# rdesc/autorally

Measured on AMD Instinct MI355X. Metric: trajectory rollouts/s per MPPI solve, higher is better.
Workload: dtype f32

## Files before the change

### autorally_amd/csrc/group_roles.hpp

```cpp
#pragma once

#include "mppi_device.hpp"
#include "noise_device.hpp"

namespace mppi {

constexpr int kGRing = 16;
constexpr int kGCtlChunk = 4;

template <class SH>
struct GroupRoles {
  static constexpr int kPose = SH::NW, kCost = SH::NW + 1, kCtl = SH::NW + 2, kRng = SH::NW + 3;
  static constexpr int kWaves = SH::NW + 4;
  static_assert(kWaves <= (int)(sizeof(SH::fin) / sizeof(int)), "fin[]");
  static_assert(SH::kR == 16 || SH::kR == 8, "rollouts per group");
};
template <class SH>
__device__ __forceinline__ int group_j(int slot) { return slot & (SH::kR - 1); }
template <class SH>
__device__ __forceinline__ bool group_real(int slot) { return slot < SH::kR; }

template <class SH>
__device__ __forceinline__ int group_seq_min(SH &sh)
{
  int m = lds_peek(lds_addr(&sh.xseq[0][0]));
#pragma unroll
  for (int w = 1; w < SH::NW; w++) m = min(m, lds_peek(lds_addr(&sh.xseq[w][0])));
  return m;
}

struct MrgHalf {
  uint32_t s0, s1, s2;
};
__device__ __forceinline__ uint32_t fold_m(uint64_t x, uint32_t C, uint32_t m)
{
  x = (x >> 32) * C + (x & 0xffffffffULL);
  x = (x >> 32) * C + (x & 0xffffffffULL);
  x = (x >> 32) * C + (x & 0xffffffffULL);
  if (x >= m) x -= m;
  return (uint32_t)x;
}
template <class SH>
__device__ __forceinline__ MrgHalf group_rng_load(const RolloutArgs &a)
{
  const int lane = threadIdx.x & 63;
  const int j = group_j<SH>((lane >> 1) & 15), c = lane & 1;
  const int k = (int)blockIdx.x * SH::kR + j;
  const int K = a.K;
  MrgHalf g{0, 0, 0};
  if (a.inline_noise != 0 && lane < 2 * kRolloutsPerWave) {
    g.s0 = a.rng_in[(3 * c) * K + k]; g.s1 = a.rng_in[(3 * c + 1) * K + k]; g.s2 = a.rng_in[(3 * c + 2) * K + k];
  }
  return g;
}
template <class SH, bool PRE = false>
__device__ __forceinline__ void group_rng_wave(const RolloutArgs &a, SH &sh, const MrgHalf pre = MrgHalf{0, 0, 0})
{
  using R = GroupRoles<SH>;
  const int lane = threadIdx.x & 63;
  const int j = group_j<SH>((lane >> 1) & 15), c = lane & 1;
  const int k = (int)blockIdx.x * SH::kR + j;
  const int K = a.K, T = a.T;
  const bool active = lane < 2 * kRolloutsPerWave;
  const bool real = lane < 2 * SH::kR;
  int budget = spin_budget_init(a.spin_budget, T, a.fault_wave == R::kRng + 1);
  if (a.inline_noise != 0) {
    const uint32_t m = c ? (uint32_t)kM2 : (uint32_t)kM1, C = c ? kC2 : kC1;
    const uint32_t A = c ? (uint32_t)kA21 : (uint32_t)kA12, Bn = c ? (uint32_t)kA23N : (uint32_t)kA13N;
    MrgHalf g{0, 0, 0};
    if constexpr (PRE) {
      g = pre;
    } else if (active) {
      g.s0 = a.rng_in[(3 * c) * K + k]; g.s1 = a.rng_in[(3 * c + 1) * K + k]; g.s2 = a.rng_in[(3 * c + 2) * K + k];
    }
    const uint32_t a_ctl = lds_addr(&sh.ctl_pub[0]);
    const uint32_t a_mypub = lds_addr(&sh.rng_pub[lane]);
    int seen = 0;
    for (int t = 0; t < T; t++) {
      float2 e = make_float2(0.5f, 0.5f);
#ifdef MPPI_DIAG_NORNG
      e = make_float2(0.25f + 0.001f * (float)t, 0.5f);
#else
#pragma unroll
      for (int d = 0; d < 2; d++) {
        const uint32_t p = fold_m((uint64_t)A * (c ? g.s2 : g.s1) + (uint64_t)Bn * (m - g.s0), C, m);
        g.s0 = g.s1; g.s1 = g.s2; g.s2 = p;
        const uint32_t p2 = (uint32_t)__builtin_amdgcn_mov_dpp((int)p, 0xB1, 0xF, 0xF, false);
        uint32_t z = (p >= p2) ? p - p2 : p + (uint32_t)kM1 - p2;
        if (z == 0) z = (uint32_t)kM1;
        const float u = (float)z * 0x1p-32f;
        if (d == 0) e.x = u; else e.y = u;
      }
#endif
      const int need = t - kGRing + 1;
      while (seen < need && --budget > 0) {
        seen = lds_peek(a_ctl);
        if (seen < need) __builtin_amdgcn_s_sleep(2);
      }
      if (active && c == 0) *reinterpret_cast<float2 *>(&sh.eps[t & (kGRing - 1)][j][0]) = e;
      lds_publish(a_mypub, t + 1);
    }
    if (real) {
      a.rng_out[(3 * c) * K + k] = g.s0; a.rng_out[(3 * c + 1) * K + k] = g.s1; a.rng_out[(3 * c + 2) * K + k] = g.s2;
    }
  }
  spin_finish(budget, lds_addr(&sh.fail[0]), lds_addr(&sh.fin[R::kRng]));
}

template <class SH>
__device__ __forceinline__ void group_control_wave(const RolloutArgs &a, SH &sh, const uint32_t a_gate_open = 0)
{
  using R = GroupRoles<SH>;
  constexpr int NSW = SH::NSW;
  static_assert(kGCtlChunk == 4 && kGRing >= 2 * kGCtlChunk, "four steps per iteration, lanes 16 q + j");
  const int lane = threadIdx.x & 63;
  const int j = group_j<SH>(lane & 15), q = lane >> 4;
  const bool real = group_real<SH>(lane & 15);
  const int k = (int)blockIdx.x * SH::kR + j;
  const int K = a.K, T = a.T;
  const bool inl = a.inline_noise != 0;
  float2 *const noise = reinterpret_cast<float2 *>(a.noise);
  const float2 *const Useq = reinterpret_cast<const float2 *>(a.U);
  const bool noise_free_k = (k == 0);
  const bool pure_noise_k = (k >= a.k99);
  const uint32_t a_cd = lds_addr(&sh.cost_done[0]);
  const uint32_t a_mypub = lds_addr(&sh.ctl_pub[lane]);
  const uint32_t a_rng = lds_addr(&sh.rng_pub[0]);
  int budget = spin_budget_init(a.spin_budget, T, a.fault_wave == R::kCtl + 1);
  const bool gated = a_gate_open != 0;
  if (gated)
    while (lds_peek(a_gate_open) == 0 && --budget > 0) __builtin_amdgcn_s_sleep(1);
  int seen_x = 0, seen_c = 0, seen_r = 0;
  for (int t0 = 0, n = 1; t0 < T; t0 += n, n = kGCtlChunk) {
    const int t = t0 + q;
    const bool live = (t < T) & (q < n);
    const int tl = live ? t : T - 1;
    float2 Ut;
    if (gated) {
      const unsigned long long ub = __hip_atomic_load(reinterpret_cast<const unsigned long long *>(Useq + tl), __ATOMIC_RELAXED, __HIP_MEMORY_SCOPE_SYSTEM);
      Ut = make_float2(__uint_as_float((unsigned)ub), __uint_as_float((unsigned)(ub >> 32)));
    } else {
      Ut = Useq[tl];
    }
    float2 e = (live && !inl) ? noise[(size_t)tl * K + k] : make_float2(0.0f, 0.0f);
    const int tm = min(t0 + n, T) - 1;
    const int need_x = (tm >= kGRing) ? (tm - kGRing) * NSW + 1 : 0;
    const int need_c = tm - kGRing + 1;
    while ((seen_x < need_x || seen_c < need_c) && --budget > 0) {
      seen_x = group_seq_min(sh);
      seen_c = lds_peek(a_cd);
      if (seen_x < need_x || seen_c < need_c) __builtin_amdgcn_s_sleep(2);
    }
    if (inl) {
      while (seen_r < tm + 1 && --budget > 0) {
        seen_r = lds_peek(a_rng);
        if (seen_r < tm + 1) __builtin_amdgcn_s_sleep(1);
      }
#ifdef MPPI_DIAG_NOBM
      e = *reinterpret_cast<const float2 *>(&sh.eps[tl & (kGRing - 1)][j][0]);
#else
      e = box_muller(*reinterpret_cast<const float2 *>(&sh.eps[tl & (kGRing - 1)][j][0]));
#endif
    }
    if (live) {
      const bool nf = noise_free_k | (t < a.opt_delay);
      const float n0 = e.x * a.nu[0], n1 = e.y * a.nu[1];
      const float du0 = nf ? 0.0f : n0, du1 = nf ? 0.0f : n1;
      float u0 = nf ? Ut.x : (pure_noise_k ? n0 : Ut.x + n0);
      float u1 = nf ? Ut.y : (pure_noise_k ? n1 : Ut.y + n1);
      if (real) noise[(size_t)t * K + k] = make_float2(u0, u1);
      u0 = clampf(u0, a.u_lo[0], a.u_hi[0]);
      u1 = clampf(u1, a.u_lo[1], a.u_hi[1]);
      const int slot = t & (kGRing - 1);
      sh.ctl_b1[slot][j] = u0;
      sh.ctl_b1[slot][kRolloutsPerWave + j] = u1;
      *reinterpret_cast<float4 *>(&sh.ctl_rec[slot][j][0]) = make_float4(u0, u1, du0, du1);
    }
    lds_publish(a_mypub, tm + 1);
  }
  spin_finish(budget, lds_addr(&sh.fail[0]), lds_addr(&sh.fin[R::kCtl]));
}

template <class SH, bool AFFINE>
__device__ __forceinline__ void group_pose_wave(const RolloutArgs &a, SH &sh)
{
  using R = GroupRoles<SH>;
  constexpr int NSW = SH::NSW;
  static_assert(SH::kR == 16, "one step per iteration: 16-rollout groups only");
  const int lane = threadIdx.x & 63;
  const int j = lane & 15;
  const int T = a.T;
  const uint32_t a_seq0 = lds_addr(&sh.xseq[0][0]);
  const uint32_t a_cd = lds_addr(&sh.cost_done[0]);
  const uint32_t a_mypub = lds_addr(&sh.pose_pub[lane]);
  float x = a.state[0], y = a.state[1], yaw = a.state[2];
  int budget = spin_budget_init(a.spin_budget, T, a.fault_wave == R::kPose + 1), seen = 0, cdone = 0;
  float tf_p = 0.0f, tb_p = 0.0f;
  for (int t = 0; t <= T; t++) {
    float tf = 0.0f, tb = 0.0f;
    if (t < T) {
      const int need = t * NSW + 1;
      while (seen < need && --budget > 0) {
        seen = SH::kRecByAll ? group_seq_min(sh) : lds_peek(a_seq0);
        if (seen < need) __builtin_amdgcn_s_sleep(1);
      }
      const float4 r0 = *reinterpret_cast<const float4 *>(&sh.rec[t & (kGRing - 1)][j][0]);
      float spsi, cpsi;
#ifdef MPPI_DIAG_NOPOSE
      spsi = 0.0f; cpsi = 1.0f; tf = x; tb = y;
#else
      sincos_fast(yaw, spsi, cpsi);
      const float st[3] = {x, y, yaw};
      track_fetch<AFFINE>(a.cost, st, cpsi, spsi, tf, tb);
#endif
      const float sd0 = fmaf(cpsi, r0.y, -(spsi * r0.z));
      const float sd1 = fmaf(spsi, r0.y, cpsi * r0.z);
      const float sd2 = a.negate_yaw_der ? -r0.w : r0.w;
      x = fmaf(sd0, a.dt, x);
      y = fmaf(sd1, a.dt, y);
      yaw = fmaf(sd2, a.dt, yaw);
    }
    if (t > 0) {
      while (cdone < t - kGRing && --budget > 0) cdone = lds_peek(a_cd);
      if (lane < kRolloutsPerWave) *reinterpret_cast<float2 *>(&sh.tex[(t - 1) & (kGRing - 1)][lane][0]) = make_float2(tf_p, tb_p);
      lds_publish(a_mypub, t);
    }
    tf_p = tf; tb_p = tb;
  }
  spin_finish(budget, lds_addr(&sh.fail[0]), lds_addr(&sh.fin[R::kPose]));
}

template <int Q>
__device__ __forceinline__ float quad_bc(float v)
{
  return __int_as_float(__builtin_amdgcn_mov_dpp(__float_as_int(v), Q * 0x55, 0xF, 0xF, false));
}
__device__ __forceinline__ void quad_chain(float v, float d, float dt, int q, float &vq, float &v_out)
{
  const float v1 = fmaf(quad_bc<0>(d), dt, v);
  const float v2 = fmaf(quad_bc<1>(d), dt, v1);
  const float v3 = fmaf(quad_bc<2>(d), dt, v2);
  v_out = fmaf(quad_bc<3>(d), dt, v3);
  const float lo = (q == 0) ? v : v1, hi = (q == 2) ? v2 : v3;
  vq = (q < 2) ? lo : hi;
}
template <class SH, bool AFFINE>
__device__ __forceinline__ void group_pose_wave4(const RolloutArgs &a, SH &sh, const float x0, const float y0, const float yaw0,
                                                 const int budget_cut = 0);
template <class SH, bool AFFINE>
__device__ __forceinline__ void group_pose_wave4(const RolloutArgs &a, SH &sh)
{
  group_pose_wave4<SH, AFFINE>(a, sh, a.state[0], a.state[1], a.state[2]);
}
template <class SH, bool AFFINE>
__device__ __forceinline__ void group_pose_wave4(const RolloutArgs &a, SH &sh, const float x0, const float y0, const float yaw0,
                                                 const int budget_cut)
{
  using R = GroupRoles<SH>;
  constexpr int NSW = SH::NSW;
  static_assert(kRolloutsPerWave == 16 && kGRing >= 8, "lane = 4 j + q");
  const int lane = threadIdx.x & 63;
  const int j = group_j<SH>(lane >> 2), q = lane & 3;
  const int T = a.T;
  const uint32_t a_seq0 = lds_addr(&sh.xseq[0][0]);
  const uint32_t a_cd = lds_addr(&sh.cost_done[0]);
  const uint32_t a_mypub = lds_addr(&sh.pose_pub[lane]);
  float x = x0, y = y0, yaw = yaw0;
  int budget = spin_budget_init(a.spin_budget, T, a.fault_wave == R::kPose + 1 || budget_cut != 0), seen = 0, cdone = 0;
  for (int t0 = 0; t0 < T; t0 += 4) {
    const int t = t0 + q;
    const int tend = min(t0 + 4, T);
    const int need = (tend - 1) * NSW + 1;
    while (seen < need && --budget > 0) {
      seen = SH::kRecByAll ? group_seq_min(sh) : lds_peek(a_seq0);
      if (seen < need) __builtin_amdgcn_s_sleep(1);
    }
    const float4 r0 = *reinterpret_cast<const float4 *>(&sh.rec[t & (kGRing - 1)][j][0]);
    float yaw_q, yaw_n, x_q, x_n, y_q, y_n;
    quad_chain(yaw, a.negate_yaw_der ? -r0.w : r0.w, a.dt, q, yaw_q, yaw_n);
    float spsi, cpsi, tf = 0.0f, tb = 0.0f;
#ifdef MPPI_DIAG_NOPOSE
    spsi = 0.0f; cpsi = 1.0f;
#else
    sincos_fast(yaw_q, spsi, cpsi);
#endif
    quad_chain(x, fmaf(cpsi, r0.y, -(spsi * r0.z)), a.dt, q, x_q, x_n);
    quad_chain(y, fmaf(spsi, r0.y, cpsi * r0.z), a.dt, q, y_q, y_n);
#ifdef MPPI_DIAG_NOPOSE
    tf = x_q; tb = y_q;
#else
    const float st[3] = {x_q, y_q, yaw_q};
    track_fetch<AFFINE>(a.cost, st, cpsi, spsi, tf, tb);
#endif
    x = x_n; y = y_n; yaw = yaw_n;
    while (cdone < tend - kGRing && --budget > 0) cdone = lds_peek(a_cd);
    if (t < T) *reinterpret_cast<float2 *>(&sh.tex[t & (kGRing - 1)][j][0]) = make_float2(tf, tb);
    lds_publish(a_mypub, tend);
  }
  spin_finish(budget, lds_addr(&sh.fail[0]), lds_addr(&sh.fin[R::kPose]));
}

template <class SH>
__device__ __forceinline__ float group_settle(SH &sh, int budget, float J)
{
  using R = GroupRoles<SH>;
  const int lane = threadIdx.x & 63;
  const uint32_t a_fin = lds_addr(&sh.fin[(lane < R::kWaves) ? lane : 0]);
  for (;;) {
    const int v = (lane == R::kCost) ? 1 : lds_peek_lanes(a_fin);
    const bool all = __builtin_amdgcn_ballot_w64(v != 0) == ~0ull;
    if (all || --budget <= 0) break;
    __builtin_amdgcn_s_sleep(1);
  }
  if (budget <= 0 || lds_peek(lds_addr(&sh.fail[0])) != 0) J = __builtin_nanf("");
  return J;
}

template <class SH, bool CTRL>
__device__ __forceinline__ void group_cost_wave(const RolloutArgs &a, SH &sh)
{
  using R = GroupRoles<SH>;
  const int lane = threadIdx.x & 63;
  static_assert(SH::kR == 16, "one step per iteration: 16-rollout groups only");
  const int j = lane & 15;
  const int k = (int)blockIdx.x * kRolloutsPerWave + j;
  const int T = a.T;
  const uint32_t a_mydone = lds_addr(&sh.cost_done[lane]);
  const uint32_t a_pose = lds_addr(&sh.pose_pub[0]);
  int crash = 0, budget = spin_budget_init(a.spin_budget, T, a.fault_wave == R::kCost + 1), seen = 0;
  float J = 0.0f;
  for (int t = 0; t < T; t++) {
    const double rt = a.inv_t[t];
    while (seen < t + 1 && --budget > 0) {
      seen = lds_peek(a_pose);
      if (seen < t + 1) __builtin_amdgcn_s_sleep(1);
    }
    const float4 r0 = *reinterpret_cast<const float4 *>(&sh.rec[t & (kGRing - 1)][j][0]);
    const float4 r1 = *reinterpret_cast<const float4 *>(&sh.ctl_rec[t & (kGRing - 1)][j][0]);
    const float2 tx = *reinterpret_cast<const float2 *>(&sh.tex[t & (kGRing - 1)][j][0]);
    lds_publish(a_mydone, t + 1);
    const int rc = (int)((t > 0) & (fabsf(r0.x) >= kRollCrash));
#ifdef MPPI_DIAG_NOCOST
    crash |= rc;
    int crash_new = crash;
    const float Jn = J + r0.y + r1.x + tx.x + (float)rt;
#else
    CostTerms ct;
    cost_terms_a<CTRL>(a.cost, a.nu, r0.y, r0.z, r1.x, r1.y, r1.z, r1.w, ct);
    crash |= rc;
    int crash_new = crash;
    const float c = cost_terms_b(a.cost, ct, tx.x, tx.y, crash_new);
    const float Jn = running_mean(J, c, t, rt);
#endif
    J = (t > 0) ? Jn : J;
    crash = (t > 0) ? crash_new : crash;
  }
  J = group_settle(sh, budget, J);
  a.costs[k] = J + 0.0f;
}

template <int Q>
__device__ __forceinline__ int quad_bc_i(int v)
{
  return __builtin_amdgcn_mov_dpp(v, Q * 0x55, 0xF, 0xF, false);
}
template <class SH, bool CTRL>
__device__ __forceinline__ void group_cost_wave4(const RolloutArgs &a, SH &sh)
{
  using R = GroupRoles<SH>;
  const int lane = threadIdx.x & 63;
  const int j = group_j<SH>(lane >> 2), q = lane & 3;
  const int k = (int)blockIdx.x * SH::kR + j;
  const int T = a.T;
  const uint32_t a_mydone = lds_addr(&sh.cost_done[lane]);
  const uint32_t a_pose = lds_addr(&sh.pose_pub[0]);
  int crash = 0, budget = spin_budget_init(a.spin_budget, T, a.fault_wave == R::kCost + 1), seen = 0;
  float J = 0.0f;
  for (int t0 = 0; t0 < T; t0 += 4) {
    const int t = t0 + q;
    const int tend = min(t0 + 4, T);
    while (seen < tend && --budget > 0) {
      seen = lds_peek(a_pose);
      if (seen < tend) __builtin_amdgcn_s_sleep(1);
    }
    const float4 r0 = *reinterpret_cast<const float4 *>(&sh.rec[t & (kGRing - 1)][j][0]);
    const float4 r1 = *reinterpret_cast<const float4 *>(&sh.ctl_rec[t & (kGRing - 1)][j][0]);
    const float2 tx = *reinterpret_cast<const float2 *>(&sh.tex[t & (kGRing - 1)][j][0]);
    lds_publish(a_mydone, tend);
    const bool counted = (t > 0) & (t < T);
    int e = (int)(fabsf(r0.x) >= kRollCrash) | (int)(tx.x >= a.cost.boundary_threshold) | (int)(tx.y >= a.cost.boundary_threshold);
    e = counted ? e : 0;
    const int c0 = crash | quad_bc_i<0>(e), c1 = c0 | quad_bc_i<1>(e), c2 = c1 | quad_bc_i<2>(e), c3 = c2 | quad_bc_i<3>(e);
    const int lo = (q == 0) ? c0 : c1, hi = (q == 2) ? c2 : c3;
    int crash_q = (q < 2) ? lo : hi;
    crash = c3;
#ifdef MPPI_DIAG_NOCOST
    const float c = r0.y + r1.x + tx.x + (float)crash_q;
#else
    CostTerms ct;
    cost_terms_a<CTRL>(a.cost, a.nu, r0.y, r0.z, r1.x, r1.y, r1.z, r1.w, ct);
    const float c = cost_terms_b(a.cost, ct, tx.x, tx.y, crash_q);
#endif
#pragma unroll
    for (int l = 0; l < 4; l++) {
      const int tl = t0 + l;
      const float cl = (l == 0) ? quad_bc<0>(c) : (l == 1) ? quad_bc<1>(c) : (l == 2) ? quad_bc<2>(c) : quad_bc<3>(c);
      if (tl > 0 && tl < T) {
#ifdef MPPI_DIAG_NOCOST
        J = J + cl + (float)a.inv_t[tl];
#else
        J = running_mean(J, cl, tl, a.inv_t[tl]);
#endif
      }
    }
  }
  J = group_settle(sh, budget, J);
  if (q == 0 && group_real<SH>(lane >> 2)) a.costs[k] = J + 0.0f;
}

}
```

### autorally_amd/csrc/mppi_device.hpp

```cpp
#pragma once

#include <hip/hip_runtime.h>
#include <stdint.h>

namespace mppi {

constexpr int kStateDim = 7;
constexpr int kControlDim = 2;
constexpr int kNetIn = 6;
constexpr int kNetOut = 4;
constexpr int kRolloutsPerWave = 16;

struct CostArgs {
  float desired_speed, speed_coeff, track_coeff, max_slip_ang, slip_penalty, track_slop;
  float crash_coeff, steering_coeff, throttle_coeff, boundary_threshold;
  float crash_cost_discounted;
  int l1_cost;
  float r_c1[3], r_c2[3], trs[3];
  int affine;
  int need_control_cost;
  int map_w, map_h;
  const float *map;
};

struct RolloutArgs {
  float state[kStateDim];
  const float *U;
  float *noise;
  float *costs;
  const float *wpack;
  const double *inv_t;
  const uint32_t *rng_in;
  uint32_t *rng_out;
  int inline_noise;
  int K, T, opt_delay, k99;
  float nu[2], u_lo[2], u_hi[2], dt;
  int negate_yaw_der;
  int spin_budget, fault_wave;
  const unsigned *gate;
  unsigned gate_seq;
  unsigned gate_ticks;
  unsigned long long *min_cost;
  unsigned min_cost_tag;
  CostArgs cost;
};
constexpr int kGateReplicas = 8;
constexpr int kGateUOffset = 16 * kGateReplicas;
inline int gate_hist_offset(int T) { return kGateUOffset + 2 * T; }
inline size_t gate_block_floats(int T) { return (size_t)gate_hist_offset(T) + 4; }
constexpr unsigned kGateCancel = 0x80000000u;

constexpr int kMinCostLines = 8, kMinCostStride = 16;
__device__ __forceinline__ unsigned cost_order_bits(float x)
{
  const unsigned b = __float_as_uint(x);
  return b ^ ((b >> 31) ? 0xFFFFFFFFu : 0x80000000u);
}
__device__ __forceinline__ float cost_from_order_bits(unsigned o)
{
  return __uint_as_float(o ^ ((o >> 31) ? 0x80000000u : 0xFFFFFFFFu));
}
template <int CTRL>
__device__ __forceinline__ float wave_dpp(float v)
{
  return __int_as_float(__builtin_amdgcn_update_dpp(0, __float_as_int(v), CTRL, 0xF, 0xF, true));
}
template <bool MIN>
__device__ __forceinline__ float wave_reduce(float v)
{
#define MPPI_RED(A, B) (MIN ? fminf((A), (B)) : (A) + (B))
  v = MPPI_RED(v, wave_dpp<0xB1>(v));
  v = MPPI_RED(v, wave_dpp<0x4E>(v));
  v = MPPI_RED(v, wave_dpp<0x141>(v));
  v = MPPI_RED(v, wave_dpp<0x140>(v));
  const auto x = __builtin_amdgcn_permlane16_swap(__float_as_uint(v), __float_as_uint(v), false, false);
  v = MPPI_RED(__uint_as_float(x[0]), __uint_as_float(x[1]));
  const auto y = __builtin_amdgcn_permlane32_swap(__float_as_uint(v), __float_as_uint(v), false, false);
  v = MPPI_RED(__uint_as_float(y[0]), __uint_as_float(y[1]));
#undef MPPI_RED
  return v;
}
__device__ __forceinline__ void publish_min_cost(const RolloutArgs &a, const float mine)
{
  if (a.min_cost == nullptr) return;
  const float m = wave_reduce<true>((mine == mine) ? mine : INFINITY);
  if ((threadIdx.x & 63) == 0 && m < INFINITY) {
    const unsigned long long key = ((unsigned long long)(~a.min_cost_tag) << 32) | cost_order_bits(m);
    (void)__hip_atomic_fetch_min(a.min_cost + (blockIdx.x % kMinCostLines) * kMinCostStride, key, __ATOMIC_RELAXED, __HIP_MEMORY_SCOPE_AGENT);
  }
}
__device__ __forceinline__ bool load_min_cost(const unsigned long long *min_cost, const unsigned tag, float &beta)
{
  if (min_cost == nullptr) return false;
  unsigned long long k[kMinCostLines];
#pragma unroll
  for (int i = 0; i < kMinCostLines; i++) k[i] = __hip_atomic_load(min_cost + i * kMinCostStride, __ATOMIC_RELAXED, __HIP_MEMORY_SCOPE_AGENT);
  unsigned long long best = k[0];
#pragma unroll
  for (int i = 1; i < kMinCostLines; i++) best = (k[i] < best) ? k[i] : best;
  beta = cost_from_order_bits((unsigned)best);
  return (unsigned)(best >> 32) == ~tag;
}

constexpr int kMaxBatch = 4;
template <int NB>
struct QuadBatchArgsT {
  int n;
  RolloutArgs inst[NB];
};
using QuadBatchArgs = QuadBatchArgsT<kMaxBatch>;
template <int NB>
inline QuadBatchArgsT<NB> batch_args_prefix(const QuadBatchArgs &b)
{
  QuadBatchArgsT<NB> s;
  s.n = b.n;
  for (int i = 0; i < NB; i++) s.inst[i] = b.inst[i];
  return s;
}
static_assert(kMaxBatch == 4, "MPPI_BATCH_DISPATCH");
#define MPPI_BATCH_DISPATCH(NB, B, BODY)     \
  do {                                      \
    if constexpr ((NB) == 2) {              \
      if (blockIdx.y == 0) BODY((B).inst[0]); \
      else BODY((B).inst[1]);               \
    } else {                                \
      switch ((int)blockIdx.y) {            \
        case 0: BODY((B).inst[0]); break;   \
        case 1: BODY((B).inst[1]); break;   \
        case 2: BODY((B).inst[2]); break;   \
        default: BODY((B).inst[3]); break;  \
      }                                     \
    }                                       \
  } while (0)

template <class T>
__device__ __forceinline__ T *load_global_ptr(T *const &field)
{
  using G = __attribute__((address_space(1))) T *;
  return (T *)*static_cast<const G *>(static_cast<const void *>(&field));
}

__device__ constexpr float kRollCrash = 1.57000005245208740234375f;
__device__ constexpr float kMinSpeed = 0.001000000047497451305389404296875f;
__device__ constexpr float kCostCapGt = 1000000061440.0f;
__device__ constexpr float kCostCap = 999999995904.0f;

__device__ __forceinline__ float clampf(float v, float lo, float hi)
{
  float r = (v > hi) ? hi : v;
  r = (v < lo) ? lo : r;
  return r;
}

__device__ __forceinline__ float tanh_fast(float x)
{
  const float e = __builtin_amdgcn_exp2f(x * 2.88539008177792681472f);
  const float r = __builtin_amdgcn_rcpf(e + 1.0f);
  return fmaf(-2.0f, r, 1.0f);
}

constexpr float kTanhScale = 2.88539008177792681472f;
__device__ __forceinline__ float tanh_bias(float z, float bs)
{
  const float e = __builtin_amdgcn_exp2f(fmaf(z, kTanhScale, bs));
  const float r = __builtin_amdgcn_rcpf(e + 1.0f);
  return fmaf(-2.0f, r, 1.0f);
}

typedef float f32x2 __attribute__((ext_vector_type(2)));
typedef float f32x4 __attribute__((ext_vector_type(4)));
__device__ __forceinline__ f32x2 tanh_bias2(f32x2 z, f32x2 bs)
{
  const f32x2 y = __builtin_elementwise_fma(z, f32x2{kTanhScale, kTanhScale}, bs);
  f32x2 e;
  e.x = __builtin_amdgcn_exp2f(y.x);
  e.y = __builtin_amdgcn_exp2f(y.y);
  const f32x2 d = e + f32x2{1.0f, 1.0f};
  f32x2 r;
  r.x = __builtin_amdgcn_rcpf(d.x);
  r.y = __builtin_amdgcn_rcpf(d.y);
  return __builtin_elementwise_fma(f32x2{-2.0f, -2.0f}, r, f32x2{1.0f, 1.0f});
}

__device__ __forceinline__ void sincos_fast(float x, float &sn, float &cs)
{
  const double xd = (double)x;
  const double q = rint(xd * 0.63661977236758134308);
  double rd = fma(-q, 1.5707963267948966, xd);
  rd = fma(-q, 6.123233995736766e-17, rd);
  const float r = (float)rd;
  const float r2 = r * r;
  const float ps = fmaf(fmaf(-1.9515295891e-4f, r2, 8.3321608736e-3f), r2, -1.6666654611e-1f);
  const float s0 = fmaf(r * r2, ps, r);
  const float pc = fmaf(fmaf(2.443315711809948e-5f, r2, -1.388731625493765e-3f), r2, 4.166664568298827e-2f);
  const float c0 = fmaf(r2 * r2, pc, fmaf(r2, -0.5f, 1.0f));
  const int qi = (int)q;
  const float a = (qi & 1) ? c0 : s0;
  const float b = (qi & 1) ? s0 : c0;
  sn = (qi & 2) ? -a : a;
  cs = ((qi + 1) & 2) ? -b : b;
}

template <bool AFFINE>
__device__ __forceinline__ unsigned texel_index(const CostArgs &c, float x, float y)
{
  float u = fmaf(c.r_c1[0], x, c.r_c2[0] * y) + c.trs[0];
  float v = fmaf(c.r_c1[1], x, c.r_c2[1] * y) + c.trs[1];
  if (!AFFINE) {
    const float w = fmaf(c.r_c1[2], x, c.r_c2[2] * y) + c.trs[2];
    u = u / w;
    v = v / w;
  }
  float fi = floorf(u * (float)c.map_w);
  float fj = floorf(v * (float)c.map_h);
  fi = fminf(fmaxf(fi, 0.0f), (float)(c.map_w - 1));
  fj = fminf(fmaxf(fj, 0.0f), (float)(c.map_h - 1));
  return (unsigned)((int)fj * c.map_w + (int)fi);
}

template <bool AFFINE>
__device__ __forceinline__ void track_fetch(const CostArgs &c, const float *s, float cpsi, float spsi,
                                            float &tf, float &tb)
{
  const float xf = fmaf(0.5f, cpsi, s[0]), yf = fmaf(0.5f, spsi, s[1]);
  const float xb = fmaf(-0.5f, cpsi, s[0]), yb = fmaf(-0.5f, spsi, s[1]);
  tf = c.map[texel_index<AFFINE>(c, xf, yf)];
  tb = c.map[texel_index<AFFINE>(c, xb, yb)];
}

struct CostTerms {
  float control_cost, speed_cost, stabilizing_cost;
};

template <bool CTRL_COST>
__device__ __forceinline__ void cost_terms_a(const CostArgs &c, const float nu[2], float s4, float s5,
                                             float u0, float u1, float du0, float du1, CostTerms &o)
{
  float control_cost = 0.0f;
  if (CTRL_COST) {
    control_cost += c.steering_coeff * du0 * (u0 - du0) / (nu[0] * nu[0]);
    control_cost += c.throttle_coeff * du1 * (u1 - du1) / (nu[1] * nu[1]);
  }
  o.control_cost = control_cost;
  const float err = s4 - c.desired_speed;
  o.speed_cost = c.speed_coeff * (c.l1_cost ? fabsf(err) : err * err);
  const float slip = -atanf(s5 / fabsf(s4));
  float stab = c.slip_penalty * (slip * slip);
  stab = (fabsf(slip) > c.max_slip_ang) ? stab + c.crash_coeff : stab;
  o.stabilizing_cost = (fabsf(s4) >= kMinSpeed) ? stab : 0.0f;
}

__device__ __forceinline__ float cost_terms_b(const CostArgs &c, const CostTerms &a, float tf, float tb,
                                              int &crash)
{
  float track_cost = (fabsf(tf) + fabsf(tb)) * 0.5f;
  track_cost = (fabsf(track_cost) < c.track_slop) ? 0.0f : c.track_coeff * track_cost;
  crash |= (int)(tf >= c.boundary_threshold) | (int)(tb >= c.boundary_threshold);
  const float crash_cost = (crash > 0) ? c.crash_cost_discounted : 0.0f;
  float cost = a.control_cost + a.speed_cost + crash_cost + track_cost + a.stabilizing_cost;
  cost = (cost >= kCostCapGt || cost != cost) ? kCostCap : cost;
  return cost;
}

template <bool CTRL_COST>
__device__ __forceinline__ float cost_finish(const CostArgs &c, const float nu[2], float s4, float s5,
                                             float tf, float tb, float u0, float u1, float du0,
                                             float du1, int &crash)
{
  CostTerms t;
  cost_terms_a<CTRL_COST>(c, nu, s4, s5, u0, u1, du0, du1, t);
  return cost_terms_b(c, t, tf, tb, crash);
}

__device__ __forceinline__ float running_mean(float J, float c, int t, double rt)
{
  const double d = (double)(c - J);
  const double td = (double)t;
  const double q0 = d * rt;
  const double e = fma(-q0, td, d);
  const double q = fma(e, rt, q0);
  return (float)((double)J + q);
}

constexpr int kSpinBudget = 1 << 22;

__device__ __forceinline__ uint32_t lds_addr(const void *p)
{
  return (uint32_t)(uintptr_t)(const __attribute__((address_space(3))) void *)p;
}
__device__ __forceinline__ void lds_publish(uint32_t addr, int v)
{
  asm volatile("ds_write_b32 %0, %1" ::"v"(addr), "v"(v) : "memory");
}
__device__ __forceinline__ void lds_put4(uint32_t addr, f32x4 v)
{
  asm volatile("ds_write_b128 %0, %1" ::"v"(addr), "v"(v) : "memory");
}
__device__ __forceinline__ int lds_peek(uint32_t addr)
{
  int v;
  asm volatile("ds_read_b32 %0, %1\n\ts_waitcnt lgkmcnt(0)" : "=&v"(v) : "v"(addr) : "memory");
  return __builtin_amdgcn_readfirstlane(v);
}
__device__ __forceinline__ void lds_pin_reads() { asm volatile("" ::: "memory"); }
__device__ __forceinline__ float row_sel(int g, float s3, float s4, float s5, float s6)
{
  const float lo = (g == 0) ? s3 : s4;
  const float hi = (g == 2) ? s5 : s6;
  return (g < 2) ? lo : hi;
}

__device__ __forceinline__ int lds_peek_lanes(uint32_t addr)
{
  int v;
  asm volatile("ds_read_b32 %0, %1\n\ts_waitcnt lgkmcnt(0)" : "=&v"(v) : "v"(addr) : "memory");
  return v;
}

__device__ __forceinline__ int spin_budget_init(int spin_budget, int T, bool inject_fault)
{
  if (inject_fault) return 0;
  return (spin_budget > 0 ? spin_budget : kSpinBudget) + 64 * T;
}
__device__ __forceinline__ void spin_finish(int budget, uint32_t a_fail, uint32_t a_fin)
{
  if (budget <= 0) lds_publish(a_fail, 1);
  lds_publish(a_fin, 1);
}

template <class SH>
__device__ __forceinline__ int group_gate_wait(const RolloutArgs &a, SH &sh)
{
  const int lane = threadIdx.x & 63;
  const unsigned *blk = a.gate + (size_t)((int)blockIdx.x % kGateReplicas) * 16;
  const unsigned long long t0 = __builtin_amdgcn_s_memrealtime();
  unsigned v = 0;
  for (;;) {
    v = __hip_atomic_load(blk + 7, __ATOMIC_RELAXED, __HIP_MEMORY_SCOPE_SYSTEM);
    if ((v & ~kGateCancel) == a.gate_seq) break;
    if (__builtin_amdgcn_s_memrealtime() - t0 > (unsigned long long)a.gate_ticks) { v = kGateCancel; break; }
    __builtin_amdgcn_s_sleep(2);
  }
  asm volatile("" ::: "memory");
  const float sv = __uint_as_float(__hip_atomic_load(blk + (lane & 7), __ATOMIC_RELAXED, __HIP_MEMORY_SCOPE_SYSTEM));
  if (lane < 7) sh.gstate[lane] = sv;
  lds_publish(lds_addr(&sh.gate_open[0]), 1);
  return (v & kGateCancel) ? 1 : 0;
}


}
```

### autorally_amd/csrc/rollout_row.hip

```cpp
#include "group_roles.hpp"
#include "mppi_kernels.hpp"

namespace mppi {

#ifdef MPPI_ROW_STAMPS
__device__ unsigned long long g_row_stamps[16];
#define RSTAMP(i)                                                                                         \
  do {                                                                                                    \
    if (blockIdx.x == 0 && (threadIdx.x & 63) == 0) {                                                     \
      unsigned long long t__;                                                                             \
      asm volatile("s_memtime %0\n\ts_waitcnt lgkmcnt(0)" : "=s"(t__)::"memory");                           \
      g_row_stamps[i] = t__;                                                                              \
    }                                                                                                     \
  } while (0)
#else
#define RSTAMP(i) do { } while (0)
#endif

template <int H>
struct RowShared {
  static constexpr int NW = 4;
  static constexpr int NSW = 1;
  static constexpr bool kRecByAll = true;
  static constexpr int kR = 16;
  int xseq[NW][64];
  float rec[kGRing][kRolloutsPerWave][4];
  int cost_done[64];
  float ctl_b1[kGRing][64];
  float ctl_rec[kGRing][kRolloutsPerWave][4];
  int ctl_pub[64];
  float tex[kGRing][kRolloutsPerWave][2];
  int pose_pub[64];
  float eps[kGRing][kRolloutsPerWave][2];
  int rng_pub[64];
  int fail[4];
  int fin[8];
  float gstate[8];
  int gate_open[8];
  float dump[NW][64 * 2 + (kGRing - 1) * kRolloutsPerWave * 4];
};

template <int H, bool TREE>
struct RowWeights {
  f32x2 w1[kNetIn], w2[H], w3[TREE ? 4 : H];
  f32x2 b1s, b2s, b3;
};

constexpr int kRowPackEntries = 40;
template <int H, bool TREE>
__device__ __forceinline__ void row_load(const float *rowpack, int p, RowWeights<H, TREE> &W)
{
  static_assert(H == 32, "entry layout of pack_row_weights");
  const float4 *pk = reinterpret_cast<const float4 *>(rowpack) + p;
#pragma unroll
  for (int i = 0; i < 3; i++) {
    const float4 v = pk[i * 16];
    W.w1[2 * i] = f32x2{v.x, v.y};
    W.w1[2 * i + 1] = f32x2{v.z, v.w};
  }
#pragma unroll
  for (int i = 0; i < H / 2; i++) {
    const float4 v = pk[(3 + i) * 16];
    W.w2[2 * i] = f32x2{v.x, v.y};
    W.w2[2 * i + 1] = f32x2{v.z, v.w};
    if constexpr (!TREE) {
      const float4 u = pk[(3 + H / 2 + i) * 16];
      W.w3[2 * i] = f32x2{u.x, u.y};
      W.w3[2 * i + 1] = f32x2{u.z, u.w};
    }
  }
  const float4 b = pk[35 * 16];
  W.b1s = f32x2{b.x, b.y};
  W.b2s = f32x2{b.z, b.w};
  if constexpr (TREE) {
    const float4 u = pk[37 * 16], v = pk[38 * 16], c = pk[39 * 16];
    W.w3[0] = f32x2{u.x, u.y};
    W.w3[1] = f32x2{u.z, u.w};
    W.w3[2] = f32x2{v.x, v.y};
    W.w3[3] = f32x2{v.z, v.w};
    W.b3 = f32x2{c.x, c.y};
  } else {
    const float4 c = pk[36 * 16];
    W.b3 = f32x2{c.x, c.y};
  }
}

template <int Q>
__device__ __forceinline__ float row_bc(float a)
{
  return __int_as_float(__builtin_amdgcn_mov_dpp(__float_as_int(a), 0x150 + Q, 0xF, 0xF, false));
}
template <int Q>
__device__ __forceinline__ f32x2 row_bc2(f32x2 a)
{
  return __builtin_bit_cast(f32x2, (long long)__builtin_amdgcn_mov_dpp(__builtin_bit_cast(long long, a), 0x150 + Q, 0xF, 0xF, false));
}
template <int Q>
__device__ __forceinline__ void row_dot_step(f32x2 &z, f32x2 &b, const f32x2 *w, f32x2 a)
{
  z = __builtin_elementwise_fma(w[2 * Q], f32x2{b.x, b.x}, z);
  __builtin_amdgcn_sched_barrier(0);
  const f32x2 bn = row_bc2<(Q + 1 < 16 ? Q + 1 : 15)>(a);
  __builtin_amdgcn_sched_barrier(0);
  z = __builtin_elementwise_fma(w[2 * Q + 1], f32x2{b.y, b.y}, z);
  __builtin_amdgcn_sched_barrier(0);
  b = bn;
}
__device__ __forceinline__ f32x2 row_dot_bc(const f32x2 *w, f32x2 a)
{
  f32x2 z = {0.0f, 0.0f};
  f32x2 b = row_bc2<0>(a);
  __builtin_amdgcn_sched_barrier(0);
#define RD4(Q) row_dot_step<Q>(z, b, w, a); row_dot_step<Q + 1>(z, b, w, a); row_dot_step<Q + 2>(z, b, w, a); row_dot_step<Q + 3>(z, b, w, a);
  RD4(0) RD4(4) RD4(8) RD4(12)
#undef RD4
  return z;
}

template <int CTRL>
__device__ __forceinline__ float dpp_add(float acc, float src)
{
  return acc + __int_as_float(__builtin_amdgcn_update_dpp(0, __float_as_int(src), CTRL, 0xF, 0xF, true));
}
__device__ __forceinline__ float row_out_tree(const f32x2 *w3, f32x2 a)
{
  const f32x2 ax = {a.x, a.x}, ay = {a.y, a.y};
  const f32x2 v01 = __builtin_elementwise_fma(w3[1], ay, w3[0] * ax);
  const f32x2 v23 = __builtin_elementwise_fma(w3[3], ay, w3[2] * ax);
  float v0 = dpp_add<0x128>(v01.x, v23.x);
  const float v1 = dpp_add<0x128>(v01.y, v23.y);
  v0 = dpp_add<0x141>(v0, v1);
  v0 = dpp_add<0xB1>(v0, v0);
  v0 = dpp_add<0x4E>(v0, v0);
  return v0;
}

template <int H, bool TREE, int Q>
__device__ __forceinline__ void row_step(const RolloutArgs &a, const RowWeights<H, TREE> &W, f32x2 &sp, f32x2 &un, const int t0,
                                         const uint32_t a_rec, const uint32_t a_myseq, const volatile int __attribute__((address_space(3))) *p_pub,
                                         const volatile f32x2 __attribute__((address_space(3))) *&pu,
                                         const volatile f32x2 __attribute__((address_space(3))) *p_u0, int &cp, int &budget)
{
  constexpr int kSlotF2 = kRolloutsPerWave * 2;
  constexpr uint32_t kRecStride = sizeof(float) * kRolloutsPerWave * 4;
  const int t = t0 + Q;
  const f32x2 u = un;
  const f32x2 slo = TREE ? f32x2{row_bc<0>(sp.x), row_bc<4>(sp.x)} : f32x2{row_bc<0>(sp.x), row_bc<0>(sp.y)};
  const f32x2 shi = TREE ? f32x2{row_bc<8>(sp.x), row_bc<12>(sp.x)} : f32x2{row_bc<1>(sp.x), row_bc<1>(sp.y)};
  if constexpr (TREE) asm volatile("ds_write_b32 %0, %1 offset:%2" ::"v"(a_rec), "v"(sp.x), "n"(Q * kRecStride) : "memory");
  else asm volatile("ds_write_b64 %0, %1 offset:%2" ::"v"(a_rec), "v"(sp), "n"(Q * kRecStride) : "memory");
  if constexpr (Q == 3) lds_publish(a_myseq, t + 1);
  f32x2 z = {0.0f, 0.0f};
  z = __builtin_elementwise_fma(W.w1[0], f32x2{slo.x, slo.x}, z);
  z = __builtin_elementwise_fma(W.w1[1], f32x2{slo.y, slo.y}, z);
  z = __builtin_elementwise_fma(W.w1[2], f32x2{shi.x, shi.x}, z);
  z = __builtin_elementwise_fma(W.w1[3], f32x2{shi.y, shi.y}, z);
  z = __builtin_elementwise_fma(W.w1[4], f32x2{u.x, u.x}, z);
  z = __builtin_elementwise_fma(W.w1[5], f32x2{u.y, u.y}, z);
  int cp_v = 0;
  if constexpr (Q == 0) cp_v = *p_pub;
  if constexpr (Q == 3) pu = p_u0 + ((t + 1) & (kGRing - 1)) * kSlotF2;
  constexpr int kUn = (Q == 3) ? 0 : (Q + 1) * kSlotF2;
  un = pu[kUn];
  const f32x2 a0 = tanh_bias2(z, W.b1s);
  const f32x2 a1 = tanh_bias2(row_dot_bc(W.w2, a0), W.b2s);
  const int want = t + 2;
  if constexpr (Q == 0) cp = __builtin_amdgcn_readfirstlane(cp_v);
  asm volatile("" : "+v"(un));
  if constexpr (TREE) {
    const float d = row_out_tree(W.w3, a1) + W.b3.x;
    sp.x = fmaf(d, a.dt, sp.x);
    asm volatile("" : "+v"(sp.x));
  } else {
    const f32x2 d = row_dot_bc(W.w3, a1) + W.b3;
    sp = __builtin_elementwise_fma(d, f32x2{a.dt, a.dt}, sp);
    asm volatile("" : "+v"(sp));
  }
  if (__builtin_expect(cp < want, 0)) {
    while (cp < want && --budget > 0) {
      cp = __builtin_amdgcn_readfirstlane(*p_pub);
      un = pu[kUn];
    }
    asm volatile("" : "+v"(un));
  }
}

template <int H, bool TREE, bool GATED = false>
__device__ __forceinline__ void row_dynamics(const RolloutArgs &a, RowShared<H> &sh, const int w)
{
  static_assert(H == 32, "row_dot_bc: 32 activations, two per lane of a 16-lane row");
  static_assert(kGRing % 4 == 0, "aligned chunks of four steps inside the ring");
  const int lane = threadIdx.x & 63;
  const int r = lane >> 4, p = lane & 15;
  const int jr = 4 * w + r;
  const bool odd = (p & 1) != 0;
  const int T = a.T;
  RowWeights<H, TREE> W;
  row_load<H, TREE>(a.wpack, p, W);
#pragma unroll
  for (int k = 0; k < H; k++) asm volatile("" : "+v"(W.w2[k]));
#pragma unroll
  for (int k = 0; k < (TREE ? 4 : H); k++) asm volatile("" : "+v"(W.w3[k]));

  const uint32_t a_myseq = lds_addr(&sh.xseq[w][lane]);
  typedef const volatile int __attribute__((address_space(3))) *lds_int_p;
  typedef const volatile f32x2 __attribute__((address_space(3))) *lds_f2_p;
  const lds_int_p p_pub = (lds_int_p)&sh.ctl_pub[0];
  uint32_t a_u0 = lds_addr(&sh.ctl_rec[0][jr][0]);
  asm volatile("" : "+v"(a_u0));
  const lds_f2_p p_u = (lds_f2_p)a_u0;
  const uint32_t a_rec0 = TREE ? (((p & 3) == 0) ? lds_addr(&sh.rec[0][jr][p >> 2]) : lds_addr(&sh.dump[w][2 * lane]))
                               : ((p < 2) ? lds_addr(&sh.rec[0][jr][2 * p]) : lds_addr(&sh.dump[w][2 * lane]));
  constexpr uint32_t kRecStride = sizeof(float) * kRolloutsPerWave * 4;

  int budget = spin_budget_init(a.spin_budget, T, a.fault_wave == w + 1);
  f32x2 sp;
  if constexpr (GATED) {
    const uint32_t a_go = lds_addr(&sh.gate_open[0]);
    while (lds_peek(a_go) == 0 && --budget > 0) __builtin_amdgcn_s_sleep(1);
    const volatile float *gs = sh.gstate;
    sp = TREE ? f32x2{gs[3 + (p >> 2)], 0.0f} : odd ? f32x2{gs[5], gs[6]} : f32x2{gs[3], gs[4]};
  } else {
    sp = TREE ? f32x2{a.state[3 + (p >> 2)], 0.0f} : odd ? f32x2{a.state[5], a.state[6]} : f32x2{a.state[3], a.state[4]};
  }
  if (w == 0) RSTAMP(2);
  int cp = 0;
  while ((cp = __builtin_amdgcn_readfirstlane(*p_pub)) < 1 && --budget > 0) __builtin_amdgcn_s_sleep(1);
  if (w == 0) RSTAMP(3);
  lds_f2_p pu = p_u;
  f32x2 un = pu[0];
  asm volatile("" : "+v"(un));

  const int NS = T - 1;
  for (int t0 = 0; t0 < NS; t0 += 4) {
    const uint32_t a_rec = a_rec0 + (uint32_t)(t0 & (kGRing - 1)) * kRecStride;
    row_step<H, TREE, 0>(a, W, sp, un, t0, a_rec, a_myseq, p_pub, pu, p_u, cp, budget);
    if (t0 + 1 >= NS) break;
    row_step<H, TREE, 1>(a, W, sp, un, t0, a_rec, a_myseq, p_pub, pu, p_u, cp, budget);
    if (t0 + 2 >= NS) break;
    row_step<H, TREE, 2>(a, W, sp, un, t0, a_rec, a_myseq, p_pub, pu, p_u, cp, budget);
    if (t0 + 3 >= NS) break;
    row_step<H, TREE, 3>(a, W, sp, un, t0, a_rec, a_myseq, p_pub, pu, p_u, cp, budget);
  }
  if (w == 0) RSTAMP(4);
  {
    const int t = T - 1;
    if constexpr (TREE) asm volatile("ds_write_b32 %0, %1" ::"v"(a_rec0 + (uint32_t)(t & (kGRing - 1)) * kRecStride), "v"(sp.x) : "memory");
    else asm volatile("ds_write_b64 %0, %1" ::"v"(a_rec0 + (uint32_t)(t & (kGRing - 1)) * kRecStride), "v"(sp) : "memory");
    lds_publish(a_myseq, t + 1);
  }
  spin_finish(budget, lds_addr(&sh.fail[0]), lds_addr(&sh.fin[w]));
}

template <int H, bool AFFINE, bool CTRL, bool TREE, bool GATED = false>
__device__ __forceinline__ void row_group(const RolloutArgs &a, RowShared<H> &sh)
{
  using SH = RowShared<H>;
  using R = GroupRoles<SH>;
  const int lane = threadIdx.x & 63;
  const int role = __builtin_amdgcn_readfirstlane(threadIdx.x >> 6);
  if (role == 0) RSTAMP(0);
  MrgHalf g0{0, 0, 0};
  if (role == R::kRng) g0 = group_rng_load<SH>(a);
  if (role == 0) {
#pragma unroll
    for (int w = 0; w < 4; w++) sh.xseq[w][lane] = 0;
    sh.cost_done[lane] = 0;
    sh.ctl_pub[lane] = 0;
    sh.pose_pub[lane] = 0;
    sh.rng_pub[lane] = 0;
    sh.fail[lane & 3] = 0;
    sh.fin[lane & 7] = 0;
    sh.gate_open[lane & 7] = 0;
  }
  __syncthreads();
  if (role == 0) RSTAMP(1);
#ifdef MPPI_ROW_RIDER_PRIO
  if (role >= 4) __builtin_amdgcn_s_setprio(MPPI_ROW_RIDER_PRIO);
#endif
  if (role < 4) row_dynamics<H, TREE, GATED>(a, sh, role);
  else if (role == R::kCost) { group_cost_wave4<SH, CTRL>(a, sh); RSTAMP(5); }
  else if (role == R::kCtl) { group_control_wave(a, sh, GATED ? lds_addr(&sh.gate_open[0]) : 0u); RSTAMP(6); }
  else if (role == R::kPose) {
    if constexpr (GATED) {
      const int shut = group_gate_wait(a, sh);
      const volatile float *gs = sh.gstate;
      const float x0 = gs[0], y0 = gs[1], yaw0 = gs[2];
      group_pose_wave4<SH, AFFINE>(a, sh, x0, y0, yaw0, shut);
    } else {
      group_pose_wave4<SH, AFFINE>(a, sh);
    }
    RSTAMP(7);
  }
  else { group_rng_wave<SH, true>(a, sh, g0); RSTAMP(8); }
}

template <int H, bool AFFINE, bool CTRL, bool TREE>
__global__ __launch_bounds__(512) void rollout_row_kernel(const RolloutArgs a)
{
  __shared__ __attribute__((aligned(16))) RowShared<H> sh;
  row_group<H, AFFINE, CTRL, TREE>(a, sh);
}
template <int H, bool AFFINE, bool CTRL, bool TREE>
__global__ __launch_bounds__(512) void rollout_row_gated_kernel(const RolloutArgs a)
{
  __shared__ __attribute__((aligned(16))) RowShared<H> sh;
  row_group<H, AFFINE, CTRL, TREE, true>(a, sh);
}

template <int H, bool AFFINE, bool CTRL, bool TREE, int NB>
__global__ __launch_bounds__(512) void rollout_row_batch_kernel(const QuadBatchArgsT<NB> b)
{
  __shared__ __attribute__((aligned(16))) RowShared<H> sh;
#define MPPI_ROW_BODY(A)                                                                                   \
  do {                                                                                                     \
    if ((int)blockIdx.x >= (A).K / kRolloutsPerWave) return;      \
    row_group<H, AFFINE, CTRL, TREE>((A), sh);                                                             \
  } while (0)
  MPPI_BATCH_DISPATCH(NB, b, MPPI_ROW_BODY);
#undef MPPI_ROW_BODY
}

template <int H, bool AFFINE, bool CTRL, bool TREE, int NB>
__global__ __launch_bounds__(512) void rollout_row_batch_gated_kernel(const QuadBatchArgsT<NB> b)
{
  __shared__ __attribute__((aligned(16))) RowShared<H> sh;
#define MPPI_ROW_BODY(A)                                                                                   \
  do {                                                                                                     \
    if ((int)blockIdx.x >= (A).K / kRolloutsPerWave) return;      \
    row_group<H, AFFINE, CTRL, TREE, true>((A), sh);                                                       \
  } while (0)
  MPPI_BATCH_DISPATCH(NB, b, MPPI_ROW_BODY);
#undef MPPI_ROW_BODY
}

bool row_variant_supported(int hidden, int n_hidden) { return hidden == 32 && n_hidden == 2; }
int row_pack_floats() { return kRowPackEntries * 16 * 4; }

#define MPPI_ROW_DISPATCH(LAUNCH, KERN, TREE, ...)                                                            \
  do {                                                                                                        \
    if (affine && !ctrl) LAUNCH((KERN<32, true, false, TREE>), __VA_ARGS__);                                  \
    else if (affine && ctrl) LAUNCH((KERN<32, true, true, TREE>), __VA_ARGS__);                               \
    else if (!affine && !ctrl) LAUNCH((KERN<32, false, false, TREE>), __VA_ARGS__);                           \
    else LAUNCH((KERN<32, false, true, TREE>), __VA_ARGS__);                                                  \
  } while (0)
#define MPPI_ROW_BATCH_DISPATCH(KERN, TREE, NB, ...)                                                                            \
  do {                                                                                                                          \
    if (affine && !ctrl) hipLaunchKernelGGL((KERN<32, true, false, TREE, NB>), __VA_ARGS__);                                    \
    else if (affine && ctrl) hipLaunchKernelGGL((KERN<32, true, true, TREE, NB>), __VA_ARGS__);                                 \
    else if (!affine && !ctrl) hipLaunchKernelGGL((KERN<32, false, false, TREE, NB>), __VA_ARGS__);                             \
    else hipLaunchKernelGGL((KERN<32, false, true, TREE, NB>), __VA_ARGS__);                                                    \
  } while (0)

hipError_t launch_rollout_row_batch(const QuadBatchArgs &b, bool tree, hipStream_t stream)
{
  if (b.n < 1 || b.n > kMaxBatch) return hipErrorInvalidValue;
  bool affine = true, ctrl = false;
  int gmax = 0;
  const bool gated = b.inst[0].gate != nullptr;
  for (int i = 0; i < b.n; i++) {
    if ((b.inst[i].gate != nullptr) != gated) return hipErrorInvalidValue;
    affine = affine && b.inst[i].cost.affine != 0;
    ctrl = ctrl || b.inst[i].cost.need_control_cost != 0;
    gmax = b.inst[i].K / kRolloutsPerWave > gmax ? b.inst[i].K / kRolloutsPerWave : gmax;
  }
  const dim3 grid(gmax, b.n), block(512);
  if (b.n <= 2) {
    const QuadBatchArgsT<2> b2 = batch_args_prefix<2>(b);
    if (gated) {
      if (tree) MPPI_ROW_BATCH_DISPATCH(rollout_row_batch_gated_kernel, true, 2, grid, block, 0, stream, b2);
      else MPPI_ROW_BATCH_DISPATCH(rollout_row_batch_gated_kernel, false, 2, grid, block, 0, stream, b2);
    } else {
      if (tree) MPPI_ROW_BATCH_DISPATCH(rollout_row_batch_kernel, true, 2, grid, block, 0, stream, b2);
      else MPPI_ROW_BATCH_DISPATCH(rollout_row_batch_kernel, false, 2, grid, block, 0, stream, b2);
    }
  } else {
    if (gated) {
      if (tree) MPPI_ROW_BATCH_DISPATCH(rollout_row_batch_gated_kernel, true, 4, grid, block, 0, stream, b);
      else MPPI_ROW_BATCH_DISPATCH(rollout_row_batch_gated_kernel, false, 4, grid, block, 0, stream, b);
    } else {
      if (tree) MPPI_ROW_BATCH_DISPATCH(rollout_row_batch_kernel, true, 4, grid, block, 0, stream, b);
      else MPPI_ROW_BATCH_DISPATCH(rollout_row_batch_kernel, false, 4, grid, block, 0, stream, b);
    }
  }
  return hipGetLastError();
}

hipError_t launch_rollout_row(int hidden, int n_hidden, const RolloutArgs &a, bool tree, hipStream_t stream)
{
  if (!row_variant_supported(hidden, n_hidden) || a.K % kRolloutsPerWave != 0) return hipErrorInvalidValue;
  const bool affine = a.cost.affine != 0, ctrl = a.cost.need_control_cost != 0;
  const dim3 grid(a.K / kRolloutsPerWave), block(512);
  if (a.gate != nullptr) {
    if (tree) MPPI_ROW_DISPATCH(MPPI_LAUNCH_ROLLOUT, rollout_row_gated_kernel, true, grid, block, 0, stream, a);
    else MPPI_ROW_DISPATCH(MPPI_LAUNCH_ROLLOUT, rollout_row_gated_kernel, false, grid, block, 0, stream, a);
    return hipGetLastError();
  }
  if (tree) MPPI_ROW_DISPATCH(MPPI_LAUNCH_ROLLOUT, rollout_row_kernel, true, grid, block, 0, stream, a);
  else MPPI_ROW_DISPATCH(MPPI_LAUNCH_ROLLOUT, rollout_row_kernel, false, grid, block, 0, stream, a);
  return hipGetLastError();
}
#undef MPPI_ROW_DISPATCH
#undef MPPI_ROW_BATCH_DISPATCH

}

#ifdef MPPI_ROW_STAMPS
extern "C" int mppi_debug_read_row_stamps(unsigned long long *out)
{
  return (int)hipMemcpyFromSymbol(out, HIP_SYMBOL(mppi::g_row_stamps), sizeof(unsigned long long) * 16);
}
#endif
```

Before: 106.8 million.

## Prefetch control-wave noise head before gate opens in gated rollout path

In the gated (persistent/graph-gated) control wave, the first 13 timesteps' Box-Muller noise is precomputed while the wave waits for the gate, then the U loads and control writes are done in a fast head burst after the gate opens. This moves the RNG-dependent latency off the critical path right after the gate opens. It adds register pressure for the head buffers and more complex spin logic, and only applies when the gated kernel variant runs. Timestamp probes are also extended.

```diff
diff --git a/autorally_amd/csrc/group_roles.hpp b/autorally_amd/csrc/group_roles.hpp
--- a/autorally_amd/csrc/group_roles.hpp
+++ b/autorally_amd/csrc/group_roles.hpp
@@ -7,6 +7,7 @@
 
 constexpr int kGRing = 16;
 constexpr int kGCtlChunk = 4;
+constexpr int kCtlHeadSteps = 13;
 
 template <class SH>
 struct GroupRoles {
@@ -107,6 +108,40 @@
   spin_finish(budget, lds_addr(&sh.fail[0]), lds_addr(&sh.fin[R::kRng]));
 }
 
+
+__device__ __forceinline__ float2 ctl_load_u_system(const float2 *p)
+{
+  const unsigned long long ub = __hip_atomic_load(reinterpret_cast<const unsigned long long *>(p), __ATOMIC_RELAXED, __HIP_MEMORY_SCOPE_SYSTEM);
+  return make_float2(__uint_as_float((unsigned)ub), __uint_as_float((unsigned)(ub >> 32)));
+}
+template <class SH>
+__device__ __forceinline__ float2 ctl_eps(SH &sh, const int tl, const int j)
+{
+#ifdef MPPI_DIAG_NOBM
+  return *reinterpret_cast<const float2 *>(&sh.eps[tl & (kGRing - 1)][j][0]);
+#else
+  return box_muller(*reinterpret_cast<const float2 *>(&sh.eps[tl & (kGRing - 1)][j][0]));
+#endif
+}
+template <class SH>
+__device__ __forceinline__ void ctl_put(const RolloutArgs &a, SH &sh, float2 *const noise, const int t, const int j, const int k, const bool real,
+                                        const bool noise_free_k, const bool pure_noise_k, const float2 Ut, const float2 e)
+{
+  const int K = a.K;
+  const bool nf = noise_free_k | (t < a.opt_delay);
+  const float n0 = e.x * a.nu[0], n1 = e.y * a.nu[1];
+  const float du0 = nf ? 0.0f : n0, du1 = nf ? 0.0f : n1;
+  float u0 = nf ? Ut.x : (pure_noise_k ? n0 : Ut.x + n0);
+  float u1 = nf ? Ut.y : (pure_noise_k ? n1 : Ut.y + n1);
+  if (real) noise[(size_t)t * K + k] = make_float2(u0, u1);
+  u0 = clampf(u0, a.u_lo[0], a.u_hi[0]);
+  u1 = clampf(u1, a.u_lo[1], a.u_hi[1]);
+  const int slot = t & (kGRing - 1);
+  sh.ctl_b1[slot][j] = u0;
+  sh.ctl_b1[slot][kRolloutsPerWave + j] = u1;
+  *reinterpret_cast<float4 *>(&sh.ctl_rec[slot][j][0]) = make_float4(u0, u1, du0, du1);
+}
+
 template <class SH>
 __device__ __forceinline__ void group_control_wave(const RolloutArgs &a, SH &sh, const uint32_t a_gate_open = 0)
 {
@@ -128,10 +163,72 @@
   const uint32_t a_rng = lds_addr(&sh.rng_pub[0]);
   int budget = spin_budget_init(a.spin_budget, T, a.fault_wave == R::kCtl + 1);
   const bool gated = a_gate_open != 0;
-  if (gated)
-    while (lds_peek(a_gate_open) == 0 && --budget > 0) __builtin_amdgcn_s_sleep(1);
   int seen_x = 0, seen_c = 0, seen_r = 0;
-  for (int t0 = 0, n = 1; t0 < T; t0 += n, n = kGCtlChunk) {
+  if (gated) {
+    constexpr int kHead = 4;
+    float2 eh[kHead], Uh[kHead];
+    int pre = 0, open = 0;
+#pragma unroll
+    for (int i = 0; i < kHead; i++) {
+      const int h0 = i ? kGCtlChunk * i - 3 : 0, hn = i ? kGCtlChunk : 1;
+      eh[i] = make_float2(0.0f, 0.0f);
+      if (inl && h0 < T && open == 0) {
+        const int t = h0 + q;
+        const int tl = ((t < T) & (q < hn)) ? t : T - 1;
+        const int tm = min(h0 + hn, T) - 1;
+        while (seen_r < tm + 1 && open == 0 && --budget > 0) {
+          seen_r = lds_peek(a_rng);
+          if (seen_r < tm + 1) {
+            open = lds_peek(a_gate_open);
+            if (open == 0) __builtin_amdgcn_s_sleep(1);
+          }
+        }
+        if (open == 0) open = lds_peek(a_gate_open);
+        if (seen_r >= tm + 1 && open == 0 && pre == i) {
+          eh[i] = ctl_eps(sh, tl, j);
+          pre = i + 1;
+        }
+      }
+    }
+    while (open == 0 && --budget > 0) {
+      open = lds_peek(a_gate_open);
+      if (open == 0) __builtin_amdgcn_s_sleep(1);
+    }
+#pragma unroll
+    for (int i = 0; i < kHead; i++) {
+      const int h0 = i ? kGCtlChunk * i - 3 : 0, hn = i ? kGCtlChunk : 1;
+      const int t = h0 + q;
+      const bool live = (t < T) & (q < hn);
+      Uh[i] = ctl_load_u_system(Useq + (live ? t : T - 1));
+      if (!inl && live) {
+        const float2 ex = noise[(size_t)t * K + k];
+        eh[i].x = ex.x;
+        eh[i].y = ex.y;
+      }
+    }
+#pragma unroll
+    for (int i = 0; i < kHead; i++) {
+      const int h0 = i ? kGCtlChunk * i - 3 : 0, hn = i ? kGCtlChunk : 1;
+      if (h0 < T) {
+        const int t = h0 + q;
+        const bool live = (t < T) & (q < hn);
+        const int tm = min(h0 + hn, T) - 1;
+        if (inl && i >= pre) {
+          while (seen_r < tm + 1 && --budget > 0) {
+            seen_r = lds_peek(a_rng);
+            if (seen_r < tm + 1) __builtin_amdgcn_s_sleep(1);
+          }
+          eh[i] = ctl_eps(sh, live ? t : T - 1, j);
+        }
+        if (live) ctl_put(a, sh, noise, t, j, k, real, noise_free_k, pure_noise_k, Uh[i], eh[i]);
+        lds_publish(a_mypub, tm + 1);
+        if (i == 0) RSTAMP(10);
+        else if (i == 1) RSTAMP(11);
+      }
+    }
+    static_assert(kGCtlChunk * kHead - 3 == kCtlHeadSteps && kCtlHeadSteps <= kGRing, "the head ends inside the first ring");
+  }
+  for (int t0 = gated ? kCtlHeadSteps : 0, n = gated ? kGCtlChunk : 1; t0 < T; t0 += n, n = kGCtlChunk) {
     const int t = t0 + q;
     const bool live = (t < T) & (q < n);
     const int tl = live ? t : T - 1;
@@ -177,6 +274,8 @@
       *reinterpret_cast<float4 *>(&sh.ctl_rec[slot][j][0]) = make_float4(u0, u1, du0, du1);
     }
     lds_publish(a_mypub, tm + 1);
+    if (tm == 0) RSTAMP(10);
+    else if (tm == 4) RSTAMP(11);
   }
   spin_finish(budget, lds_addr(&sh.fail[0]), lds_addr(&sh.fin[R::kCtl]));
 }
diff --git a/autorally_amd/csrc/mppi_device.hpp b/autorally_amd/csrc/mppi_device.hpp
--- a/autorally_amd/csrc/mppi_device.hpp
+++ b/autorally_amd/csrc/mppi_device.hpp
@@ -282,6 +282,10 @@
   return (float)((double)J + q);
 }
 
+#ifndef RSTAMP
+#define RSTAMP(i) do { } while (0)
+#endif
+
 constexpr int kSpinBudget = 1 << 22;
 
 __device__ __forceinline__ uint32_t lds_addr(const void *p)
diff --git a/autorally_amd/csrc/rollout_row.hip b/autorally_amd/csrc/rollout_row.hip
--- a/autorally_amd/csrc/rollout_row.hip
+++ b/autorally_amd/csrc/rollout_row.hip
@@ -1,21 +1,21 @@
-#include "group_roles.hpp"
-#include "mppi_kernels.hpp"
-
+#ifdef MPPI_ROW_STAMPS
 namespace mppi {
-
-#ifdef MPPI_ROW_STAMPS
 __device__ unsigned long long g_row_stamps[16];
+}
 #define RSTAMP(i)                                                                                         \
   do {                                                                                                    \
-    if (blockIdx.x == 0 && (threadIdx.x & 63) == 0) {                                                     \
+    if (blockIdx.x == 0 && blockIdx.y == 0 && (threadIdx.x & 63) == 0) {                                  \
       unsigned long long t__;                                                                             \
       asm volatile("s_memtime %0\n\ts_waitcnt lgkmcnt(0)" : "=s"(t__)::"memory");                           \
       g_row_stamps[i] = t__;                                                                              \
     }                                                                                                     \
   } while (0)
-#else
-#define RSTAMP(i) do { } while (0)
 #endif
+
+#include "group_roles.hpp"
+#include "mppi_kernels.hpp"
+
+namespace mppi {
 
 template <int H>
 struct RowShared {
@@ -235,12 +235,18 @@
   for (int t0 = 0; t0 < NS; t0 += 4) {
     const uint32_t a_rec = a_rec0 + (uint32_t)(t0 & (kGRing - 1)) * kRecStride;
     row_step<H, TREE, 0>(a, W, sp, un, t0, a_rec, a_myseq, p_pub, pu, p_u, cp, budget);
+#ifdef MPPI_ROW_STAMPS
+    if (w == 0 && t0 == 0) RSTAMP(12);
+#endif
     if (t0 + 1 >= NS) break;
     row_step<H, TREE, 1>(a, W, sp, un, t0, a_rec, a_myseq, p_pub, pu, p_u, cp, budget);
     if (t0 + 2 >= NS) break;
     row_step<H, TREE, 2>(a, W, sp, un, t0, a_rec, a_myseq, p_pub, pu, p_u, cp, budget);
     if (t0 + 3 >= NS) break;
     row_step<H, TREE, 3>(a, W, sp, un, t0, a_rec, a_myseq, p_pub, pu, p_u, cp, budget);
+#ifdef MPPI_ROW_STAMPS
+    if (w == 0 && t0 == 0) RSTAMP(13);
+#endif
   }
   if (w == 0) RSTAMP(4);
   {
@@ -284,6 +290,7 @@
   else if (role == R::kPose) {
     if constexpr (GATED) {
       const int shut = group_gate_wait(a, sh);
+      RSTAMP(9);
       const volatile float *gs = sh.gstate;
       const float x0 = gs[0], y0 = gs[1], yaw0 = gs[2];
       group_pose_wave4<SH, AFFINE>(a, sh, x0, y0, yaw0, shut);
```

Result: faster. 108.7 million (median of 6 runs) (+1.8%).
